# ubisoft/ubisoft-laforge-daft-exprt

Measured on AMD Instinct MI355X. Metric: training mel-frames/sec, higher is better.
Workload: dtype bf16; 1 GPU; BASELINE configs[1]: full Daft-Exprt train step (fwd + 7-term loss + bwd + Adam, dropout on, adversarial weight at max), 11 speakers, batch 48 per GPU, 80-bin mel, 1<=T<=1000 (utterance 0 = 1000 frames), bf16 MFMA operands, fp32 accumulate/master; global_batch=48, batch_per_gpu=48, accumulation_steps=1, parallelism=dp1, params=14727153

## Files before the change

### ubisoft-laforge-daft-exprt_amd/csrc/upsample.hip

```cpp
#include "dx_common.h"

namespace {

constexpr int D = 128;
constexpr float LOG_SQRT_2PI = 0.91893853320467274178f;

struct PrepArgs {
  const float* enc; const float* dur_f; const float* energy; const float* pitch; const int64_t* lengths;
  const float* w_dur; const float* b_dur; const float* w_en; const float* b_en; const float* w_pi; const float* b_pi;
  const float* w_r; const float* b_r;
  float* xp; float* ranges; float* r_pre; float* rin;
  int L; long rows;
};
__device__ __forceinline__ float conv3(const float* ft, int l, int L, const float* w) {
  const float xm = l > 0 ? ft[l - 1] : 0.f, x0 = ft[l], xq = l + 1 < L ? ft[l + 1] : 0.f;
  return w[0] * xm + w[1] * x0 + w[2] * xq;
}
__global__ __launch_bounds__(256) void gu_prepare_kernel(PrepArgs a) {
  const int lane = threadIdx.x & 63;
  const long row = (long)blockIdx.x * 4 + (threadIdx.x >> 6);
  if (row >= a.rows) return;
  const int b = (int)(row / a.L), l = (int)(row - (long)b * a.L);
  float acc = 0.f;
#pragma unroll
  for (int k = 0; k < 2; ++k) {
    const int c = lane * 2 + k;
    const float xp = a.enc[row * D + c] + conv3(a.energy + (long)b * a.L, l, a.L, a.w_en + c * 3) + a.b_en[c] +
                     conv3(a.pitch + (long)b * a.L, l, a.L, a.w_pi + c * 3) + a.b_pi[c];
    a.xp[row * D + c] = xp;
    const float rin = xp + conv3(a.dur_f + (long)b * a.L, l, a.L, a.w_dur + c * 3) + a.b_dur[c];
    if (a.rin) a.rin[row * D + c] = rin;
    acc += rin * a.w_r[c];
  }
  acc = dx_wave_sum(acc) + a.b_r[0];
  if (lane == 0) {
    const bool pad = l >= (int)a.lengths[b];
    const float sp = acc > 20.f ? acc : log1pf(expf(acc));
    a.ranges[row] = pad ? 1.f : sp;
    if (a.r_pre) a.r_pre[row] = acc;
  }
}

__global__ __launch_bounds__(64) void gu_means_kernel(const int64_t* __restrict__ dur_int, float* __restrict__ means,
                                                       int64_t* __restrict__ totals, int B, int L) {
  const int b = blockIdx.x, lane = threadIdx.x;
  long long carry = 0;
  for (int l0 = 0; l0 < L; l0 += 64) {
    const int l = l0 + lane;
    const long long d = l < L ? (long long)dur_int[(long)b * L + l] : 0;
    const long long incl = dx_wave_scan(d, lane);
    const long long excl = carry + incl - d;
    if (l < L) {
      float mu = (float)d / 2.f;
      if (l > 0) mu += (float)excl;
      means[(long)b * L + l] = mu;
    }
    carry += __shfl(incl, 63, 64);
  }
  if (lane == 0) totals[b] = carry;
}

struct UpArgs {
  const float* xp; const float* ranges; const float* means; const int64_t* in_len; const int64_t* out_len;
  const float* pos;
  float* weights;
  float* out;
  int L, T;
};
constexpr int TT = 32;
constexpr int LC = 64;

__global__ __launch_bounds__(256) void gu_upsample_fwd_kernel(UpArgs a) {
  __shared__ float Wt[LC][TT + 1];
  __shared__ float part[8][TT];
  __shared__ float denom[TT];
  __shared__ int lrange[2];
  const int tid = threadIdx.x, b = blockIdx.y, t0 = blockIdx.x * TT;
  if (tid == 0) { lrange[0] = 1 << 30; lrange[1] = -1; }
  __syncthreads();
  const int tt = tid & 31, lg = tid >> 5;
  const int L = a.L, T = a.T;
  const int len = (int)a.in_len[b];
  const float tc = (float)(t0 + tt) + 0.5f;
  const float* mu = a.means + (long)b * L;
  const float* sg = a.ranges + (long)b * L;
  float s = 0.f;
  int lo = 1 << 30, hi = -1;
  for (int l = lg; l < len; l += 8) {
    const float sd = sg[l], dlt = tc - mu[l];
    const float pv = expf(-(dlt * dlt) / (2.f * sd * sd) - logf(sd) - LOG_SQRT_2PI);
    s += pv;
    if (pv != 0.f) { lo = min(lo, l); hi = max(hi, l); }
  }
  part[lg][tt] = s;
  if (hi >= 0) { atomicMin(&lrange[0], lo); atomicMax(&lrange[1], hi); }
  __syncthreads();
  if (tid < TT) {
    float d = 0.f;
#pragma unroll
    for (int k = 0; k < 8; ++k) d += part[k][tid];
    denom[tid] = d + 1e-20f;
  }
  __syncthreads();
  const int ft = tid >> 3, cg = tid & 7;
  float acc[16];
#pragma unroll
  for (int i = 0; i < 16; ++i) acc[i] = 0.f;
  const float den = denom[tt];
  for (int l0 = 0; l0 < L; l0 += LC) {
    for (int l = l0 + lg; l < min(L, l0 + LC); l += 8) {
      float w = 0.f;
      if (l < len) {
        const float sd = sg[l], dlt = tc - mu[l];
        w = expf(-(dlt * dlt) / (2.f * sd * sd) - logf(sd) - LOG_SQRT_2PI) / den;
      }
      Wt[l - l0][tt] = w;
      if (t0 + tt < T) a.weights[((long)b * L + l) * T + t0 + tt] = w;
    }
    __syncthreads();
    const int lmax = min(min(min(L, l0 + LC), len), lrange[1] + 1);
    for (int l = max(l0, lrange[0]); l < lmax; ++l) {
      const float w = Wt[l - l0][ft];
      const f32x4* xr = reinterpret_cast<const f32x4*>(a.xp + ((long)b * L + l) * D + cg * 16);
#pragma unroll
      for (int v = 0; v < 4; ++v) {
        const f32x4 x = xr[v];
        acc[v * 4 + 0] = fmaf(w, x[0], acc[v * 4 + 0]); acc[v * 4 + 1] = fmaf(w, x[1], acc[v * 4 + 1]);
        acc[v * 4 + 2] = fmaf(w, x[2], acc[v * 4 + 2]); acc[v * 4 + 3] = fmaf(w, x[3], acc[v * 4 + 3]);
      }
    }
    __syncthreads();
  }
  const int t = t0 + ft;
  if (t < T) {
    float* o = a.out + ((long)b * T + t) * D + cg * 16;
    if (a.pos) {
      const bool valid = t < (int)a.out_len[b];
      const float* pr = a.pos + (long)t * D + cg * 16;
#pragma unroll
      for (int i = 0; i < 16; ++i) o[i] = valid ? acc[i] + pr[i] : 0.f;
    } else {
#pragma unroll
      for (int i = 0; i < 16; ++i) o[i] = acc[i];
    }
  }
}

struct UpBwd1Args {
  const float* g;
  const float* xp; const float* weights; const int64_t* in_len; const int64_t* out_len;
  float* dw;
  float* dsum;
  int L, T;
};
__global__ __launch_bounds__(256) void gu_upsample_bwd1_kernel(UpBwd1Args a) {
  __shared__ float G[TT][D + 1];
  __shared__ float part[8][TT];
  __shared__ int lrange[2];
  const int tid = threadIdx.x, b = blockIdx.y, t0 = blockIdx.x * TT;
  const int L = a.L, T = a.T, len = (int)a.in_len[b];
  const int tvalid = a.out_len ? (int)a.out_len[b] : T;
  if (tid == 0) { lrange[0] = 1 << 30; lrange[1] = -1; }
  __syncthreads();
  {
    const int tt = tid & 31, lg = tid >> 5;
    int lo = 1 << 30, hi = -1;
    if (t0 + tt < T)
      for (int l = lg; l < len; l += 8)
        if (a.weights[((long)b * L + l) * T + t0 + tt] != 0.f) { lo = min(lo, l); hi = max(hi, l); }
    if (hi >= 0) { atomicMin(&lrange[0], lo); atomicMax(&lrange[1], hi); }
  }
  for (int i = tid; i < TT * D; i += 256) {
    const int r = i / D, c = i - r * D, t = t0 + r;
    G[r][c] = (t < T && t < tvalid) ? a.g[((long)b * T + t) * D + c] : 0.f;
  }
  __syncthreads();
  const int tt = tid & 31, lg = tid >> 5;
  float dacc = 0.f;
  const int lfirst = lrange[0], llast = min(lrange[1], len - 1);
  for (int l = lfirst + lg; l <= llast; l += 8) {
    float dot = 0.f;
    {
      const float* xr = a.xp + ((long)b * L + l) * D;
      for (int c = 0; c < D; ++c) dot = fmaf(G[tt][c], xr[c], dot);
    }
    if (t0 + tt < T) {
      const long idx = ((long)b * L + l) * T + t0 + tt;
      a.dw[idx] = dot;
      dacc += a.weights[idx] * dot;
    }
  }
  part[lg][tt] = dacc;
  __syncthreads();
  if (tid < TT && t0 + tid < T) {
    float d = 0.f;
#pragma unroll
    for (int k = 0; k < 8; ++k) d += part[k][tid];
    a.dsum[(long)b * T + t0 + tid] = d;
  }
}

struct UpBwd2Args {
  const float* g; const float* weights; const float* dw; const float* dsum; const float* means; const float* ranges;
  const float* r_pre; const float* w_r; const int64_t* in_len; const int64_t* out_len;
  float* dxp;
  float* drin;
  float* dr;
  int L, T;
};
__global__ __launch_bounds__(128) void gu_upsample_bwd2_kernel(UpBwd2Args a) {
  __shared__ float red[2];
  const int c = threadIdx.x, l = blockIdx.x, b = blockIdx.y;
  const int L = a.L, T = a.T, len = (int)a.in_len[b];
  const long row = (long)b * L + l;
  float* dxp = a.dxp + row * D;
  float* drin = a.drin + row * D;
  if (l >= len) {
    dxp[c] = 0.f; drin[c] = 0.f;
    if (c == 0) a.dr[row] = 0.f;
    return;
  }
  const int tvalid = min(T, a.out_len ? (int)a.out_len[b] : T);
  const float* w = a.weights + row * T;
  const float* dwr = a.dw + row * T;
  const float* ds = a.dsum + (long)b * T;
  const float mu = a.means[row], sd = a.ranges[row];
  __shared__ int trange[2];
  if (c == 0) { trange[0] = 1 << 30; trange[1] = -1; }
  __syncthreads();
  {
    int lo = 1 << 30, hi = -1;
    for (int t = c; t < tvalid; t += 128) if (w[t] != 0.f) { lo = min(lo, t); hi = max(hi, t); }
    if (hi >= 0) { atomicMin(&trange[0], lo); atomicMax(&trange[1], hi); }
  }
  __syncthreads();
  const int tfirst = trange[0], tlast = trange[1];
  float acc = 0.f, dsig = 0.f;
  for (int t = tfirst; t <= tlast; ++t) acc = fmaf(w[t], a.g[((long)b * T + t) * D + c], acc);
  for (int t = tfirst + c; t <= tlast; t += 128) {
    const float wt = w[t];
    if (wt != 0.f) {
      const float dlt = (float)t + 0.5f - mu;
      dsig += wt * (dwr[t] - ds[t]) * (dlt * dlt / (sd * sd * sd) - 1.f / sd);
    }
  }
  dsig = dx_wave_sum(dsig);
  if ((c & 63) == 0) red[c >> 6] = dsig;
  __syncthreads();
  const float rp = a.r_pre[row];
  const float dr = (red[0] + red[1]) * (rp > 20.f ? 1.f : 1.f / (1.f + expf(-rp)));
  const float dri = dr * a.w_r[c];
  dxp[c] = acc + dri;
  drin[c] = dri;
  if (c == 0) a.dr[row] = dr;
}

}

extern "C" int dx_gu_prepare(const float* enc, const float* dur_float, const float* energy, const float* pitch,
                             const int64_t* in_lengths, const float* w_dur, const float* b_dur, const float* w_en,
                             const float* b_en, const float* w_pi, const float* b_pi, const float* w_range,
                             const float* b_range, float* xp, float* ranges, float* r_pre, float* rin, int B, int L,
                             int C, void* stream) {
  DX_REQUIRE(enc && dur_float && energy && pitch && in_lengths && xp && ranges, DX_ERR_ARG, "dx_gu_prepare: null pointer");
  DX_REQUIRE(C == D, DX_ERR_UNSUPPORTED, "dx_gu_prepare: C=%d (only 128)", C);
  DX_REQUIRE(B > 0 && L > 0, DX_ERR_SHAPE, "dx_gu_prepare: empty shape");
  PrepArgs a{enc, dur_float, energy, pitch, in_lengths, w_dur, b_dur, w_en, b_en, w_pi, b_pi, w_range, b_range, xp, ranges, r_pre, rin, L, (long)B * L};
  hipLaunchKernelGGL(gu_prepare_kernel, dim3((unsigned)((a.rows + 3) / 4)), dim3(256), 0, (hipStream_t)stream, a);
  DX_LAUNCH_CHECK();
  return DX_OK;
}

extern "C" int dx_gu_means(const int64_t* durations_int, float* means, int64_t* totals, int B, int L, void* stream) {
  DX_REQUIRE(durations_int && means && totals, DX_ERR_ARG, "dx_gu_means: null pointer");
  hipLaunchKernelGGL(gu_means_kernel, dim3(B), dim3(64), 0, (hipStream_t)stream, durations_int, means, totals, B, L);
  DX_LAUNCH_CHECK();
  return DX_OK;
}

extern "C" int dx_gu_upsample_fwd(const float* xp, const float* ranges, const float* means, const int64_t* in_lengths,
                                  const int64_t* out_lengths, const float* pos_table, float* weights, float* out, int B,
                                  int L, int T, int C, void* stream) {
  DX_REQUIRE(xp && ranges && means && in_lengths && weights && out, DX_ERR_ARG, "dx_gu_upsample_fwd: null pointer");
  DX_REQUIRE(!pos_table || out_lengths, DX_ERR_ARG, "dx_gu_upsample_fwd: pos_table needs out_lengths");
  DX_REQUIRE(C == D, DX_ERR_UNSUPPORTED, "dx_gu_upsample_fwd: C=%d (only 128)", C);
  DX_REQUIRE(B > 0 && L > 0 && T > 0, DX_ERR_SHAPE, "dx_gu_upsample_fwd: empty shape");
  UpArgs a{xp, ranges, means, in_lengths, out_lengths, pos_table, weights, out, L, T};
  hipLaunchKernelGGL(gu_upsample_fwd_kernel, dim3(dx_cdiv(T, TT), B), dim3(256), 0, (hipStream_t)stream, a);
  DX_LAUNCH_CHECK();
  return DX_OK;
}

extern "C" int dx_gu_upsample_bwd(const float* g, const float* xp, const float* weights, const float* means,
                                  const float* ranges, const float* r_pre, const float* w_range,
                                  const int64_t* in_lengths, const int64_t* out_lengths, float* dw_ws, float* dsum_ws,
                                  float* dxp, float* drin, float* dr, int B, int L, int T, int C, void* stream) {
  DX_REQUIRE(g && xp && weights && means && ranges && r_pre && w_range && in_lengths && dw_ws && dsum_ws && dxp && drin && dr,
             DX_ERR_ARG, "dx_gu_upsample_bwd: null pointer");
  DX_REQUIRE(C == D, DX_ERR_UNSUPPORTED, "dx_gu_upsample_bwd: C=%d (only 128)", C);
  hipStream_t s = (hipStream_t)stream;
  UpBwd1Args a1{g, xp, weights, in_lengths, out_lengths, dw_ws, dsum_ws, L, T};
  hipLaunchKernelGGL(gu_upsample_bwd1_kernel, dim3(dx_cdiv(T, TT), B), dim3(256), 0, s, a1);
  UpBwd2Args a2{g, weights, dw_ws, dsum_ws, means, ranges, r_pre, w_range, in_lengths, out_lengths, dxp, drin, dr, L, T};
  hipLaunchKernelGGL(gu_upsample_bwd2_kernel, dim3(L, B), dim3(128), 0, s, a2);
  DX_LAUNCH_CHECK();
  return DX_OK;
}
```

Before: 4.843 million mel-frames/s.

## Skip out-of-reach Gaussian tokens via analytic support bounds in upsampling kernels

Computes an analytic support interval for each token's Gaussian, the range beyond which its weight underflows to zero in fp32. Each frame tile compacts the tokens that can reach it into a shared list and evaluates exp and the weighted sum only for those, instead of scanning all L tokens with atomics to find the range. Backward kernels reuse the same compaction and support bounds in place of scanning the weights tensor. bwd2 is widened to 256 threads with vectorised gradient loads and a block reduction. This adds more shared memory, spill paths to global memory when more than GU_CAP tokens are live, and correctness depends on the underflow bound being conservative.

```diff
diff --git a/ubisoft-laforge-daft-exprt_amd/csrc/upsample.hip b/ubisoft-laforge-daft-exprt_amd/csrc/upsample.hip
--- a/ubisoft-laforge-daft-exprt_amd/csrc/upsample.hip
+++ b/ubisoft-laforge-daft-exprt_amd/csrc/upsample.hip
@@ -60,6 +60,47 @@
   if (lane == 0) totals[b] = carry;
 }
 
+constexpr float GU_QZERO = 106.f;
+__device__ __forceinline__ void gu_reach(float mu, float sd, float logsd, int& lo, int& hi) {
+  const float r = sd * sqrtf(2.f * fmaxf(GU_QZERO - logsd, 0.f)) * 1.001f + 1.f;
+  const float c = mu - 0.5f;
+  if (sd > 0.f && r < 1e9f && fabsf(c) < 1e9f) {
+    lo = (int)floorf(c - r);
+    hi = (int)ceilf(c + r);
+  } else {
+    lo = -2147483647 - 1;
+    hi = 2147483647;
+  }
+}
+
+constexpr int TT = 32;
+constexpr int GU_R = 256;
+constexpr int GU_CAP = 128;
+
+struct GuList {
+  int l[GU_R];
+  float mu[GU_R], h[GU_R], logsd[GU_R];
+  int in[GU_R];
+  int part[4];
+};
+__device__ __forceinline__ int gu_compact(GuList& s, const float* __restrict__ mu, const float* __restrict__ sg, int l0, int len, int t0, int t1) {
+  const int tid = threadIdx.x, l = l0 + tid;
+  int in = 0;
+  float m = 0.f, sd = 1.f, lsd = 0.f;
+  if (l < len) {
+    m = mu[l]; sd = sg[l]; lsd = logf(sd);
+    int lo, hi;
+    gu_reach(m, sd, lsd, lo, hi);
+    in = (lo <= t1 && hi >= t0) ? 1 : 0;
+  }
+  s.in[tid] = in;
+  int n = 0;
+  const int pos = dx_block_scan_step<4>(in, n, s.part);
+  if (in) { s.l[pos] = l; s.mu[pos] = m; s.h[pos] = 2.f * sd * sd; s.logsd[pos] = lsd; }
+  __syncthreads();
+  return n;
+}
+
 struct UpArgs {
   const float* xp; const float* ranges; const float* means; const int64_t* in_len; const int64_t* out_len;
   const float* pos;
@@ -67,33 +108,40 @@
   float* out;
   int L, T;
 };
-constexpr int TT = 32;
-constexpr int LC = 64;
-
-__global__ __launch_bounds__(256) void gu_upsample_fwd_kernel(UpArgs a) {
-  __shared__ float Wt[LC][TT + 1];
+
+__global__ __launch_bounds__(256) __attribute__((amdgpu_waves_per_eu(6))) void gu_upsample_fwd_kernel(UpArgs a) {
+  __shared__ GuList ls;
+  __shared__ float Wt[GU_CAP][TT + 1];
   __shared__ float part[8][TT];
   __shared__ float denom[TT];
-  __shared__ int lrange[2];
   const int tid = threadIdx.x, b = blockIdx.y, t0 = blockIdx.x * TT;
-  if (tid == 0) { lrange[0] = 1 << 30; lrange[1] = -1; }
-  __syncthreads();
   const int tt = tid & 31, lg = tid >> 5;
   const int L = a.L, T = a.T;
-  const int len = (int)a.in_len[b];
+  const int len = (int)dx_clamp_len(a.in_len, b, L);
+  const int t1 = min(t0 + TT, T) - 1;
+  const bool tin = t0 + tt < T;
   const float tc = (float)(t0 + tt) + 0.5f;
   const float* mu = a.means + (long)b * L;
   const float* sg = a.ranges + (long)b * L;
+  float* wcol = a.weights + (long)b * L * T + t0 + tt;
   float s = 0.f;
-  int lo = 1 << 30, hi = -1;
-  for (int l = lg; l < len; l += 8) {
-    const float sd = sg[l], dlt = tc - mu[l];
-    const float pv = expf(-(dlt * dlt) / (2.f * sd * sd) - logf(sd) - LOG_SQRT_2PI);
-    s += pv;
-    if (pv != 0.f) { lo = min(lo, l); hi = max(hi, l); }
+  int base = 0, n = 0;
+  for (int l0 = 0; l0 < len; l0 += GU_R) {
+    n = gu_compact(ls, mu, sg, l0, len, t0, t1);
+    for (int j = 0; j < n; ++j) {
+      const int l = ls.l[j];
+      if ((l & 7) == lg) {
+        const float dlt = tc - ls.mu[j];
+        const float pv = expf(-(dlt * dlt) / ls.h[j] - ls.logsd[j] - LOG_SQRT_2PI);
+        s += pv;
+        if (base + j < GU_CAP) Wt[base + j][tt] = pv;
+        else if (tin) wcol[(long)l * T] = pv;
+      }
+    }
+    base += n;
+    __syncthreads();
   }
   part[lg][tt] = s;
-  if (hi >= 0) { atomicMin(&lrange[0], lo); atomicMax(&lrange[1], hi); }
   __syncthreads();
   if (tid < TT) {
     float d = 0.f;
@@ -103,92 +151,113 @@
   }
   __syncthreads();
   const int ft = tid >> 3, cg = tid & 7;
-  float acc[16];
-#pragma unroll
-  for (int i = 0; i < 16; ++i) acc[i] = 0.f;
+  f32x4 acc[4];
+#pragma unroll
+  for (int v = 0; v < 4; ++v) acc[v] = f32x4{0.f, 0.f, 0.f, 0.f};
   const float den = denom[tt];
-  for (int l0 = 0; l0 < L; l0 += LC) {
-    for (int l = l0 + lg; l < min(L, l0 + LC); l += 8) {
-      float w = 0.f;
-      if (l < len) {
-        const float sd = sg[l], dlt = tc - mu[l];
-        w = expf(-(dlt * dlt) / (2.f * sd * sd) - logf(sd) - LOG_SQRT_2PI) / den;
-      }
-      Wt[l - l0][tt] = w;
-      if (t0 + tt < T) a.weights[((long)b * L + l) * T + t0 + tt] = w;
-    }
+  const bool one_round = len <= GU_R;
+  const bool valid = a.pos ? t0 + ft < (int)a.out_len[b] : true;
+  base = 0;
+  for (int l0 = 0; l0 < L; l0 += GU_R) {
+    const bool live = l0 < len;
+    if (live) {
+      if (!one_round) n = gu_compact(ls, mu, sg, l0, len, t0, t1);
+      for (int j = 0; j < n; ++j) {
+        const int l = ls.l[j];
+        if ((l & 7) == lg) {
+          if (base + j < GU_CAP) Wt[base + j][tt] = Wt[base + j][tt] / den;
+          else if (tin) wcol[(long)l * T] = wcol[(long)l * T] / den;
+        }
+      }
+      __syncthreads();
+#pragma unroll 2
+      for (int j = 0; j < n; ++j) {
+        const int l = ls.l[j];
+        float w;
+        if (base + j < GU_CAP) w = Wt[base + j][ft];
+        else w = t0 + ft < T ? a.weights[((long)b * L + l) * T + t0 + ft] : 0.f;
+        const f32x4* xr = reinterpret_cast<const f32x4*>(a.xp + ((long)b * L + l) * D) + cg;
+#pragma unroll
+        for (int v = 0; v < 4; ++v) {
+          const f32x4 x = xr[v * 8];
+          acc[v][0] = fmaf(w, x[0], acc[v][0]); acc[v][1] = fmaf(w, x[1], acc[v][1]);
+          acc[v][2] = fmaf(w, x[2], acc[v][2]); acc[v][3] = fmaf(w, x[3], acc[v][3]);
+        }
+      }
+    }
+    if (l0 + GU_R >= L && t0 + ft < T) {
+      const int t = t0 + ft;
+      f32x4* o = reinterpret_cast<f32x4*>(a.out + ((long)b * T + t) * D) + cg;
+      if (a.pos) {
+        const f32x4* pr = reinterpret_cast<const f32x4*>(a.pos + (long)t * D) + cg;
+        f32x4 p[4];
+#pragma unroll
+        for (int v = 0; v < 4; ++v) p[v] = pr[v * 8];
+#pragma unroll
+        for (int v = 0; v < 4; ++v) o[v * 8] = valid ? acc[v] + p[v] : f32x4{0.f, 0.f, 0.f, 0.f};
+      } else {
+#pragma unroll
+        for (int v = 0; v < 4; ++v) o[v * 8] = acc[v];
+      }
+    }
+    if (tin) {
+      if (live)
+        for (int j = 0; j < n; ++j) {
+          const int l = ls.l[j];
+          if ((l & 7) == lg && base + j < GU_CAP) wcol[(long)l * T] = Wt[base + j][tt];
+        }
+      const int lend = min(L, l0 + GU_R);
+      for (int l = l0 + lg; l < lend; l += 8)
+        if (!(live && ls.in[l - l0])) wcol[(long)l * T] = 0.f;
+    }
+    if (live) base += n;
     __syncthreads();
-    const int lmax = min(min(min(L, l0 + LC), len), lrange[1] + 1);
-    for (int l = max(l0, lrange[0]); l < lmax; ++l) {
-      const float w = Wt[l - l0][ft];
-      const f32x4* xr = reinterpret_cast<const f32x4*>(a.xp + ((long)b * L + l) * D + cg * 16);
-#pragma unroll
-      for (int v = 0; v < 4; ++v) {
-        const f32x4 x = xr[v];
-        acc[v * 4 + 0] = fmaf(w, x[0], acc[v * 4 + 0]); acc[v * 4 + 1] = fmaf(w, x[1], acc[v * 4 + 1]);
-        acc[v * 4 + 2] = fmaf(w, x[2], acc[v * 4 + 2]); acc[v * 4 + 3] = fmaf(w, x[3], acc[v * 4 + 3]);
-      }
-    }
-    __syncthreads();
-  }
-  const int t = t0 + ft;
-  if (t < T) {
-    float* o = a.out + ((long)b * T + t) * D + cg * 16;
-    if (a.pos) {
-      const bool valid = t < (int)a.out_len[b];
-      const float* pr = a.pos + (long)t * D + cg * 16;
-#pragma unroll
-      for (int i = 0; i < 16; ++i) o[i] = valid ? acc[i] + pr[i] : 0.f;
-    } else {
-#pragma unroll
-      for (int i = 0; i < 16; ++i) o[i] = acc[i];
-    }
   }
 }
 
 struct UpBwd1Args {
   const float* g;
-  const float* xp; const float* weights; const int64_t* in_len; const int64_t* out_len;
+  const float* xp; const float* weights; const float* means; const float* ranges; const int64_t* in_len; const int64_t* out_len;
   float* dw;
   float* dsum;
   int L, T;
 };
 __global__ __launch_bounds__(256) void gu_upsample_bwd1_kernel(UpBwd1Args a) {
+  __shared__ GuList ls;
   __shared__ float G[TT][D + 1];
   __shared__ float part[8][TT];
-  __shared__ int lrange[2];
   const int tid = threadIdx.x, b = blockIdx.y, t0 = blockIdx.x * TT;
-  const int L = a.L, T = a.T, len = (int)a.in_len[b];
-  const int tvalid = a.out_len ? (int)a.out_len[b] : T;
-  if (tid == 0) { lrange[0] = 1 << 30; lrange[1] = -1; }
-  __syncthreads();
-  {
-    const int tt = tid & 31, lg = tid >> 5;
-    int lo = 1 << 30, hi = -1;
-    if (t0 + tt < T)
-      for (int l = lg; l < len; l += 8)
-        if (a.weights[((long)b * L + l) * T + t0 + tt] != 0.f) { lo = min(lo, l); hi = max(hi, l); }
-    if (hi >= 0) { atomicMin(&lrange[0], lo); atomicMax(&lrange[1], hi); }
+  const int L = a.L, T = a.T, len = (int)dx_clamp_len(a.in_len, b, L);
+  const int tvalid = a.out_len ? (int)dx_clamp_len(a.out_len, b, T) : T;
+  if (t0 >= tvalid) {
+    if (tid < TT && t0 + tid < T) a.dsum[(long)b * T + t0 + tid] = 0.f;
+    return;
   }
   for (int i = tid; i < TT * D; i += 256) {
     const int r = i / D, c = i - r * D, t = t0 + r;
-    G[r][c] = (t < T && t < tvalid) ? a.g[((long)b * T + t) * D + c] : 0.f;
-  }
-  __syncthreads();
+    G[r][c] = t < tvalid ? a.g[((long)b * T + t) * D + c] : 0.f;
+  }
   const int tt = tid & 31, lg = tid >> 5;
+  const int t1 = min(t0 + TT, T) - 1;
   float dacc = 0.f;
-  const int lfirst = lrange[0], llast = min(lrange[1], len - 1);
-  for (int l = lfirst + lg; l <= llast; l += 8) {
-    float dot = 0.f;
-    {
-      const float* xr = a.xp + ((long)b * L + l) * D;
-      for (int c = 0; c < D; ++c) dot = fmaf(G[tt][c], xr[c], dot);
-    }
-    if (t0 + tt < T) {
-      const long idx = ((long)b * L + l) * T + t0 + tt;
-      a.dw[idx] = dot;
-      dacc += a.weights[idx] * dot;
-    }
+  for (int l0 = 0; l0 < len; l0 += GU_R) {
+    const int n = gu_compact(ls, a.means + (long)b * L, a.ranges + (long)b * L, l0, len, t0, t1);
+    for (int j = lg; j < n; j += 8) {
+      const int l = ls.l[j];
+      const f32x4* xr = reinterpret_cast<const f32x4*>(a.xp + ((long)b * L + l) * D);
+      float dot = 0.f;
+      for (int c4 = 0; c4 < D / 4; ++c4) {
+        const f32x4 x = xr[c4];
+        dot = fmaf(G[tt][c4 * 4 + 0], x[0], dot); dot = fmaf(G[tt][c4 * 4 + 1], x[1], dot);
+        dot = fmaf(G[tt][c4 * 4 + 2], x[2], dot); dot = fmaf(G[tt][c4 * 4 + 3], x[3], dot);
+      }
+      if (t0 + tt < T) {
+        const long idx = ((long)b * L + l) * T + t0 + tt;
+        a.dw[idx] = dot;
+        dacc += a.weights[idx] * dot;
+      }
+    }
+    __syncthreads();
   }
   part[lg][tt] = dacc;
   __syncthreads();
@@ -208,51 +277,58 @@
   float* dr;
   int L, T;
 };
-__global__ __launch_bounds__(128) void gu_upsample_bwd2_kernel(UpBwd2Args a) {
-  __shared__ float red[2];
-  const int c = threadIdx.x, l = blockIdx.x, b = blockIdx.y;
-  const int L = a.L, T = a.T, len = (int)a.in_len[b];
+__global__ __launch_bounds__(256) void gu_upsample_bwd2_kernel(UpBwd2Args a) {
+  __shared__ float racc[8][D];
+  __shared__ float red[4];
+  const int tid = threadIdx.x, l = blockIdx.x, b = blockIdx.y;
+  const int L = a.L, T = a.T, len = (int)dx_clamp_len(a.in_len, b, L);
   const long row = (long)b * L + l;
   float* dxp = a.dxp + row * D;
   float* drin = a.drin + row * D;
+  const int tvalid = a.out_len ? (int)dx_clamp_len(a.out_len, b, T) : T;
+  const float mu = a.means[row], sd = a.ranges[row], rp = a.r_pre[row], wr = a.w_r[tid & (D - 1)];
   if (l >= len) {
-    dxp[c] = 0.f; drin[c] = 0.f;
-    if (c == 0) a.dr[row] = 0.f;
+    if (tid < D) { dxp[tid] = 0.f; drin[tid] = 0.f; }
+    if (tid == 0) a.dr[row] = 0.f;
     return;
   }
-  const int tvalid = min(T, a.out_len ? (int)a.out_len[b] : T);
   const float* w = a.weights + row * T;
   const float* dwr = a.dw + row * T;
   const float* ds = a.dsum + (long)b * T;
-  const float mu = a.means[row], sd = a.ranges[row];
-  __shared__ int trange[2];
-  if (c == 0) { trange[0] = 1 << 30; trange[1] = -1; }
-  __syncthreads();
-  {
-    int lo = 1 << 30, hi = -1;
-    for (int t = c; t < tvalid; t += 128) if (w[t] != 0.f) { lo = min(lo, t); hi = max(hi, t); }
-    if (hi >= 0) { atomicMin(&trange[0], lo); atomicMax(&trange[1], hi); }
-  }
-  __syncthreads();
-  const int tfirst = trange[0], tlast = trange[1];
-  float acc = 0.f, dsig = 0.f;
-  for (int t = tfirst; t <= tlast; ++t) acc = fmaf(w[t], a.g[((long)b * T + t) * D + c], acc);
-  for (int t = tfirst + c; t <= tlast; t += 128) {
+  int lo, hi;
+  gu_reach(mu, sd, logf(sd), lo, hi);
+  const int tfirst = max(lo, 0), tlast = min(hi, tvalid - 1);
+  const int fg = tid >> 5, cq = tid & 31;
+  f32x4 acc = {0.f, 0.f, 0.f, 0.f};
+  const float* gb = a.g + (long)b * T * D + cq * 4;
+#pragma unroll 2
+  for (int t = tfirst + fg; t <= tlast; t += 8) {
+    const float wt = w[t];
+    const f32x4 gv = *reinterpret_cast<const f32x4*>(gb + (long)t * D);
+    acc[0] = fmaf(wt, gv[0], acc[0]); acc[1] = fmaf(wt, gv[1], acc[1]);
+    acc[2] = fmaf(wt, gv[2], acc[2]); acc[3] = fmaf(wt, gv[3], acc[3]);
+  }
+  float dsig = 0.f;
+  for (int t = tfirst + tid; t <= tlast; t += 256) {
     const float wt = w[t];
     if (wt != 0.f) {
       const float dlt = (float)t + 0.5f - mu;
       dsig += wt * (dwr[t] - ds[t]) * (dlt * dlt / (sd * sd * sd) - 1.f / sd);
     }
   }
-  dsig = dx_wave_sum(dsig);
-  if ((c & 63) == 0) red[c >> 6] = dsig;
-  __syncthreads();
-  const float rp = a.r_pre[row];
-  const float dr = (red[0] + red[1]) * (rp > 20.f ? 1.f : 1.f / (1.f + expf(-rp)));
-  const float dri = dr * a.w_r[c];
-  dxp[c] = acc + dri;
-  drin[c] = dri;
-  if (c == 0) a.dr[row] = dr;
+#pragma unroll
+  for (int i = 0; i < 4; ++i) racc[fg][cq * 4 + i] = acc[i];
+  dsig = dx_block_sum<4, false>(dsig, red);
+  if (tid < D) {
+    float s = 0.f;
+#pragma unroll
+    for (int k = 0; k < 8; ++k) s += racc[k][tid];
+    const float dr = dsig * (rp > 20.f ? 1.f : 1.f / (1.f + expf(-rp)));
+    const float dri = dr * wr;
+    dxp[tid] = s + dri;
+    drin[tid] = dri;
+    if (tid == 0) a.dr[row] = dr;
+  }
 }
 
 }
@@ -299,10 +375,10 @@
              DX_ERR_ARG, "dx_gu_upsample_bwd: null pointer");
   DX_REQUIRE(C == D, DX_ERR_UNSUPPORTED, "dx_gu_upsample_bwd: C=%d (only 128)", C);
   hipStream_t s = (hipStream_t)stream;
-  UpBwd1Args a1{g, xp, weights, in_lengths, out_lengths, dw_ws, dsum_ws, L, T};
+  UpBwd1Args a1{g, xp, weights, means, ranges, in_lengths, out_lengths, dw_ws, dsum_ws, L, T};
   hipLaunchKernelGGL(gu_upsample_bwd1_kernel, dim3(dx_cdiv(T, TT), B), dim3(256), 0, s, a1);
   UpBwd2Args a2{g, weights, dw_ws, dsum_ws, means, ranges, r_pre, w_range, in_lengths, out_lengths, dxp, drin, dr, L, T};
-  hipLaunchKernelGGL(gu_upsample_bwd2_kernel, dim3(L, B), dim3(128), 0, s, a2);
+  hipLaunchKernelGGL(gu_upsample_bwd2_kernel, dim3(L, B), dim3(256), 0, s, a2);
   DX_LAUNCH_CHECK();
   return DX_OK;
 }
```

Result: faster. 4.899 million mel-frames/s (median of 6 runs) (+1.2%).
